# tenpy/tenpy

Hardware: NVIDIA H100
Metric: dmrg_two_site_sweep_wall_clock (lower is better)
Workload: dtype f64

## Files before the change

tenpy_b200/csrc/common.cuh:

```cuda
#pragma once
#include <cuda_runtime.h>
#include <stdint.h>
#include <stdio.h>
#include <atomic>
#include <string>

#include "../../include/b200npc.h"

namespace b200 {

extern thread_local std::string g_last_error;
int set_error(int code, const char *fmt, ...);

#define B200_CUDA_CHECK(expr)                                                                        \
    do {                                                                                             \
        cudaError_t _e = (expr);                                                                     \
        if (_e != cudaSuccess)                                                                       \
            return b200::set_error(B200_ERR_CUDA, "%s failed at %s:%d: %s", #expr, __FILE__, __LINE__, \
                                   cudaGetErrorString(_e));                                          \
    } while (0)

#define B200_CHECK_LAUNCH()                                                                          \
    do {                                                                                             \
        b200::g_kernel_launches.fetch_add(1, std::memory_order_relaxed);                             \
        cudaError_t _e = cudaGetLastError();                                                         \
        if (_e != cudaSuccess)                                                                       \
            return b200::set_error(B200_ERR_CUDA, "kernel launch failed at %s:%d: %s", __FILE__,       \
                                   __LINE__, cudaGetErrorString(_e));                                \
    } while (0)

int sm_count();
extern std::atomic<long long> g_kernel_launches;

#ifndef B200_DMMA_K4
#define B200_DMMA_K4 0
#endif

__device__ __forceinline__ void dmma_m8n8k4(double &c0, double &c1, double a, double b) {
    asm volatile("mma.sync.aligned.m8n8k4.row.col.f64.f64.f64.f64 {%0,%1}, {%2}, {%3}, {%0,%1};\n"
                 : "+d"(c0), "+d"(c1)
                 : "d"(a), "d"(b));
}

__device__ __forceinline__ void dmma_16x8x8_k4(double (&c)[4], const double (&a)[4], const double (&b)[2]) {
    dmma_m8n8k4(c[0], c[1], a[0], b[0]);
    dmma_m8n8k4(c[0], c[1], a[2], b[1]);
    dmma_m8n8k4(c[2], c[3], a[1], b[0]);
    dmma_m8n8k4(c[2], c[3], a[3], b[1]);
}

__device__ __forceinline__ void dmma_16x8x8_k8(double (&c)[4], const double (&a)[4], const double (&b)[2]) {
    asm volatile(
        "mma.sync.aligned.m16n8k8.row.col.f64.f64.f64.f64 {%0,%1,%2,%3}, {%4,%5,%6,%7}, {%8,%9}, "
        "{%0,%1,%2,%3};\n"
        : "+d"(c[0]), "+d"(c[1]), "+d"(c[2]), "+d"(c[3])
        : "d"(a[0]), "d"(a[1]), "d"(a[2]), "d"(a[3]), "d"(b[0]), "d"(b[1]));
}

__device__ __forceinline__ void dmma_16x8x8(double (&c)[4], const double (&a)[4], const double (&b)[2]) {
#if B200_DMMA_K4
    dmma_16x8x8_k4(c, a, b);
#else
    dmma_16x8x8_k8(c, a, b);
#endif
}

__device__ __forceinline__ uint32_t smem_u32(const void *p) {
    return static_cast<uint32_t>(__cvta_generic_to_shared(p));
}
__device__ __forceinline__ void cp_async16(void *smem_dst, const void *gsrc, int src_bytes) {
    asm volatile("cp.async.cg.shared.global [%0], [%1], 16, %2;\n" ::"r"(smem_u32(smem_dst)), "l"(gsrc),
                 "r"(src_bytes));
}
__device__ __forceinline__ void cp_async8(void *smem_dst, const void *gsrc, int src_bytes) {
    asm volatile("cp.async.ca.shared.global [%0], [%1], 8, %2;\n" ::"r"(smem_u32(smem_dst)), "l"(gsrc),
                 "r"(src_bytes));
}
__device__ __forceinline__ void cp_async_commit() { asm volatile("cp.async.commit_group;\n" ::); }
template <int N>
__device__ __forceinline__ void cp_async_wait() {
    asm volatile("cp.async.wait_group %0;\n" ::"n"(N));
}

__device__ __forceinline__ double warp_sum(double v) {
#pragma unroll
    for (int o = 16; o > 0; o >>= 1) v += __shfl_xor_sync(0xffffffffu, v, o);
    return v;
}
__device__ __forceinline__ double warp_max(double v) {
#pragma unroll
    for (int o = 16; o > 0; o >>= 1) v = fmax(v, __shfl_xor_sync(0xffffffffu, v, o));
    return v;
}
__device__ __forceinline__ double block_sum(double v, double *red) {
    v = warp_sum(v);
    int lane = threadIdx.x & 31, w = threadIdx.x >> 5;
    if (lane == 0) red[w] = v;
    __syncthreads();
    int nw = (blockDim.x + 31) >> 5;
    double r = 0.0;
    if (w == 0) {
        r = (lane < nw) ? red[lane] : 0.0;
        r = warp_sum(r);
    }
    __syncthreads();
    return r;
}

}
```

tenpy_b200/csrc/gemm.cu:

```cuda
#include <algorithm>
#include <cstdarg>
#include <cstring>
#include <numeric>
#include <vector>

#include "common.cuh"

namespace b200 {

thread_local std::string g_last_error;
std::atomic<long long> g_kernel_launches{0};

int set_error(int code, const char *fmt, ...) {
    char buf[1024];
    va_list ap;
    va_start(ap, fmt);
    vsnprintf(buf, sizeof(buf), fmt, ap);
    va_end(ap);
    g_last_error = buf;
    return code;
}

int sm_count() {
    static int cached = -1;
    if (cached < 0) {
        int dev = 0, n = 0;
        if (cudaGetDevice(&dev) == cudaSuccess &&
            cudaDeviceGetAttribute(&n, cudaDevAttrMultiProcessorCount, dev) == cudaSuccess)
            cached = n;
        else
            return 132;
    }
    return cached;
}

struct GemmTask {
    int64_t c_off;
    int32_t m, n;
    int32_t pair_begin, pair_end;
};
struct GemmPair {
    int64_t a_off, b_off;
    int32_t k, pad;
};
struct GemmTile {
    int32_t task, tm, tn, pad;
};

constexpr int GEMM_BK = 16;
constexpr int GEMM_STAGES = 3;

template <int BM, int BN>
constexpr int gemm_smem_bytes() {
    return GEMM_STAGES * (BM * (GEMM_BK + 4) + GEMM_BK * (BN + 4)) * (int)sizeof(double);
}

template <int BM, int BN, int WARPS_M, int WARPS_N, bool VEC>
__global__ void __launch_bounds__(WARPS_M *WARPS_N * 32)
    grouped_gemm_kernel(const double *__restrict__ A, const double *__restrict__ B, double *__restrict__ C,
                        const GemmTile *__restrict__ tiles, const GemmTask *__restrict__ tasks,
                        const GemmPair *__restrict__ pairs) {
    constexpr int BK = GEMM_BK, STAGES = GEMM_STAGES;
    constexpr int NTHR = WARPS_M * WARPS_N * 32;
    constexpr int WM = BM / WARPS_M, WN = BN / WARPS_N;
    constexpr int MT = WM / 16, NTL = WN / 8;
    constexpr int LDA_S = BK + 4, LDB_S = BN + 4;
    static_assert(WM % 16 == 0 && WN % 8 == 0, "warp tile");

    extern __shared__ __align__(16) double smem[];
    double *As = smem;
    double *Bs = smem + STAGES * BM * LDA_S;

    const GemmTile tile = tiles[blockIdx.x];
    const GemmTask task = tasks[tile.task];
    const int m = task.m, n = task.n;
    const int row0 = tile.tm * BM, col0 = tile.tn * BN;
    const int tid = threadIdx.x, lane = tid & 31, warp = tid >> 5;
    const int warp_m = warp / WARPS_N, warp_n = warp % WARPS_N;
    const int g = lane >> 2, t = lane & 3;

    int total = 0;
    for (int p = task.pair_begin; p < task.pair_end; ++p) total += (pairs[p].k + BK - 1) / BK;

    int pp = task.pair_begin, pk = 0;
    GemmPair cur = (pp < task.pair_end) ? pairs[pp] : GemmPair{0, 0, 0, 0};

    auto load_stage = [&](int stage) {
        const int k = cur.k;
        const int kbase = pk * BK;
// ... 46 lines not shown
            ++pp;
            if (pp < task.pair_end) cur = pairs[pp];
        }
    };

    double acc[MT][NTL][4];
#pragma unroll
    for (int i = 0; i < MT; ++i)
#pragma unroll
        for (int j = 0; j < NTL; ++j)
#pragma unroll
            for (int e = 0; e < 4; ++e) acc[i][j][e] = 0.0;

    int loaded = 0;
#pragma unroll
    for (int s = 0; s < STAGES - 1; ++s) {
        if (loaded < total) {
            load_stage(s);
            ++loaded;
        }
        cp_async_commit();
    }

    for (int it = 0; it < total; ++it) {
        cp_async_wait<STAGES - 2>();
        __syncthreads();
        if (loaded < total) {
            load_stage((it + STAGES - 1) % STAGES);
            ++loaded;
        }
        cp_async_commit();

        const double *as = As + (it % STAGES) * BM * LDA_S + (warp_m * WM) * LDA_S;
        const double *bs = Bs + (it % STAGES) * BK * LDB_S + warp_n * WN;
#pragma unroll
        for (int kk = 0; kk < BK; kk += 8) {
            double af[MT][4], bf[NTL][2];
#pragma unroll
            for (int i = 0; i < MT; ++i) {
                const double *ap = as + (i * 16 + g) * LDA_S + kk + t;
                af[i][0] = ap[0];
                af[i][1] = ap[8 * LDA_S];
                af[i][2] = ap[4];
                af[i][3] = ap[8 * LDA_S + 4];
            }
#pragma unroll
            for (int j = 0; j < NTL; ++j) {
                const double *bp = bs + (kk + t) * LDB_S + j * 8 + g;
                bf[j][0] = bp[0];
                bf[j][1] = bp[4 * LDB_S];
            }
#pragma unroll
            for (int i = 0; i < MT; ++i)
#pragma unroll
                for (int j = 0; j < NTL; ++j) dmma_16x8x8(acc[i][j], af[i], bf[j]);
        }
    }
    cp_async_wait<0>();

    double *cg = C + task.c_off;
#pragma unroll
    for (int i = 0; i < MT; ++i) {
#pragma unroll
        for (int j = 0; j < NTL; ++j) {
            int r = row0 + warp_m * WM + i * 16 + g;
            int c = col0 + warp_n * WN + j * 8 + 2 * t;
#pragma unroll
            for (int h = 0; h < 2; ++h) {
                int rr = r + 8 * h;
                if (rr < m) {
                    double *dst = cg + (int64_t)rr * n + c;
                    if (VEC) {
                        if (c < n) *reinterpret_cast<double2 *>(dst) = make_double2(acc[i][j][2 * h], acc[i][j][2 * h + 1]);
                    } else {
                        if (c < n) dst[0] = acc[i][j][2 * h];
                        if (c + 1 < n) dst[1] = acc[i][j][2 * h + 1];
                    }
                }
            }
        }
    }
}

constexpr int THIN_MAX = 8;
constexpr int THIN_KSUM = 64;
constexpr int THIN_ROWS = 256;

__global__ void __launch_bounds__(THIN_ROWS)
    thin_n_kernel(const double *__restrict__ A, const double *__restrict__ B, double *__restrict__ C,
                  const GemmTile *__restrict__ tiles, const GemmTask *__restrict__ tasks, const GemmPair *__restrict__ pairs) {
    const GemmTile tile = tiles[blockIdx.x];
    const GemmTask task = tasks[tile.task];
    const int64_t r = (int64_t)tile.tm * THIN_ROWS + threadIdx.x;
    if (r >= task.m) return;
    const int n = task.n;
    double acc[THIN_MAX];
#pragma unroll
    for (int j = 0; j < THIN_MAX; ++j) acc[j] = 0.0;
    for (int p = task.pair_begin; p < task.pair_end; ++p) {
        const GemmPair pr = pairs[p];
        const double *a = A + pr.a_off + r * pr.k;
        const double *b = B + pr.b_off;
        for (int kk = 0; kk < pr.k; ++kk) {
            const double av = a[kk];
#pragma unroll
            for (int j = 0; j < THIN_MAX; ++j)
                if (j < n) acc[j] = fma(av, __ldg(b + (int64_t)kk * n + j), acc[j]);
        }
    }
    double *c = C + task.c_off + r * n;
#pragma unroll
    for (int j = 0; j < THIN_MAX; ++j)
        if (j < n) c[j] = acc[j];
}

__global__ void __launch_bounds__(THIN_ROWS)
    thin_m_kernel(const double *__restrict__ A, const double *__restrict__ B, double *__restrict__ C,
                  const GemmTile *__restrict__ tiles, const GemmTask *__restrict__ tasks, const GemmPair *__restrict__ pairs) {
    const GemmTile tile = tiles[blockIdx.x];
    const GemmTask task = tasks[tile.task];
    const int64_t col = (int64_t)tile.tn * THIN_ROWS + threadIdx.x;
    if (col >= task.n) return;
    const int m = task.m, n = task.n;
    double acc[THIN_MAX];
#pragma unroll
    for (int i = 0; i < THIN_MAX; ++i) acc[i] = 0.0;
    for (int p = task.pair_begin; p < task.pair_end; ++p) {
        const GemmPair pr = pairs[p];
        const double *a = A + pr.a_off;
        const double *b = B + pr.b_off + col;
        for (int kk = 0; kk < pr.k; ++kk) {
            const double bv = b[(int64_t)kk * n];
#pragma unroll
            for (int i = 0; i < THIN_MAX; ++i)
                if (i < m) acc[i] = fma(__ldg(a + (int64_t)i * pr.k + kk), bv, acc[i]);
        }
    }
    double *c = C + task.c_off + col;
#pragma unroll
    for (int i = 0; i < THIN_MAX; ++i)
        if (i < m) c[(int64_t)i * n] = acc[i];
}

struct TileSet {
    std::vector<GemmTile> tiles[5];
};

static inline int64_t cdiv(int64_t a, int64_t b) { return (a + b - 1) / b; }

static void build_tiles(const std::vector<GemmTask> &tasks, const std::vector<GemmPair> &pairs, TileSet &ts) {
    struct Key {
        int64_t work;
        GemmTile tile;
    };
    std::vector<Key> keyed[5];
    static const int force_cfg = getenv("B200_GEMM_FORCE_CFG") ? atoi(getenv("B200_GEMM_FORCE_CFG")) : -1;
    for (size_t ti = 0; ti < tasks.size(); ++ti) {
        const GemmTask &tk = tasks[ti];
        if (tk.m <= 0 || tk.n <= 0) continue;
        int64_t ksum = 0;
        for (int p = tk.pair_begin; p < tk.pair_end; ++p) ksum += pairs[p].k;
        int64_t area128 = cdiv(tk.m, 128) * cdiv(tk.n, 128) * 128 * 128;
        int64_t area64 = cdiv(tk.m, 64) * cdiv(tk.n, 64) * 64 * 64;
        int64_t area32 = cdiv(tk.m, 32) * cdiv(tk.n, 32) * 32 * 32;
        (void)area128;
        int cfg = 1;
        if (area32 * 10 < area64 * 7) cfg = 2;
        if (force_cfg >= 0) cfg = force_cfg;
        if (force_cfg < 0 && ksum <= THIN_KSUM) {
            if (tk.n <= THIN_MAX && tk.m >= 4 * tk.n) cfg = 3;
            else if (tk.m <= THIN_MAX && tk.n >= 4 * tk.m) cfg = 4;
        }
        if (cfg >= 3) {
            int64_t nt = cdiv(cfg == 3 ? tk.m : tk.n, THIN_ROWS);
            for (int64_t i = 0; i < nt; ++i) {
                Key k;
                k.work = ksum;
                k.tile = cfg == 3 ? GemmTile{(int32_t)ti, (int32_t)i, 0, 0} : GemmTile{(int32_t)ti, 0, (int32_t)i, 0};
                keyed[cfg].push_back(k);
            }
            continue;
        }
        int b = cfg == 0 ? 128 : (cfg == 1 ? 64 : 32);
        for (int tm = 0; tm < cdiv(tk.m, b); ++tm)
            for (int tn = 0; tn < cdiv(tk.n, b); ++tn) {
                Key k;
                k.work = ksum;
                k.tile = GemmTile{(int32_t)ti, tm, tn, 0};
                keyed[cfg].push_back(k);
            }
    }
    for (int c = 0; c < 5; ++c) {
        std::stable_sort(keyed[c].begin(), keyed[c].end(), [](const Key &x, const Key &y) { return x.work > y.work; });
        ts.tiles[c].clear();
        for (auto &k : keyed[c]) ts.tiles[c].push_back(k.tile);
    }
}

struct DeviceGemmDesc {
    GemmTask *tasks = nullptr;
    GemmPair *pairs = nullptr;
    GemmTile *tiles[5] = {nullptr, nullptr, nullptr, nullptr, nullptr};
    int n_tiles[5] = {0, 0, 0, 0, 0};
    bool vec = false;
    int device = -1;
    void release() {
        if (tasks) cudaFree(tasks);
        if (pairs) cudaFree(pairs);
        for (int c = 0; c < 5; ++c) {
            if (tiles[c]) cudaFree(tiles[c]);
            tiles[c] = nullptr;
        }
        tasks = nullptr;
        pairs = nullptr;
    }
};

static int upload_desc(const std::vector<GemmTask> &tasks, const std::vector<GemmPair> &pairs, DeviceGemmDesc &d) {
    TileSet ts;
    build_tiles(tasks, pairs, ts);
    B200_CUDA_CHECK(cudaGetDevice(&d.device));
    if (!tasks.empty()) {
        B200_CUDA_CHECK(cudaMalloc(&d.tasks, tasks.size() * sizeof(GemmTask)));
        B200_CUDA_CHECK(cudaMemcpy(d.tasks, tasks.data(), tasks.size() * sizeof(GemmTask), cudaMemcpyHostToDevice));
    }
    if (!pairs.empty()) {
        B200_CUDA_CHECK(cudaMalloc(&d.pairs, pairs.size() * sizeof(GemmPair)));
        B200_CUDA_CHECK(cudaMemcpy(d.pairs, pairs.data(), pairs.size() * sizeof(GemmPair), cudaMemcpyHostToDevice));
    }
    for (int c = 0; c < 5; ++c) {
        d.n_tiles[c] = (int)ts.tiles[c].size();
        if (d.n_tiles[c]) {
            B200_CUDA_CHECK(cudaMalloc(&d.tiles[c], ts.tiles[c].size() * sizeof(GemmTile)));
            B200_CUDA_CHECK(cudaMemcpy(d.tiles[c], ts.tiles[c].data(), ts.tiles[c].size() * sizeof(GemmTile),
                                       cudaMemcpyHostToDevice));
        }
    }
    bool vec = true;
    for (auto &t : tasks)
        if ((t.n & 1) || (t.c_off & 1)) vec = false;
    for (auto &p : pairs)
        if ((p.k & 1) || (p.a_off & 1) || (p.b_off & 1)) vec = false;
    d.vec = vec;
    return B200_OK;
}

template <int BM, int BN, int WMW, int WNW, bool VEC>
static int launch_cfg(const DeviceGemmDesc &d, int cfg, const double *A, const double *B, double *C, cudaStream_t st) {
    if (d.n_tiles[cfg] == 0) return B200_OK;
    auto kern = grouped_gemm_kernel<BM, BN, WMW, WNW, VEC>;
    constexpr int smem = gemm_smem_bytes<BM, BN>();
    static bool attr_set = false;
    if (!attr_set) {
        B200_CUDA_CHECK(cudaFuncSetAttribute(kern, cudaFuncAttributeMaxDynamicSharedMemorySize, smem));
        attr_set = true;
    }
    kern<<<d.n_tiles[cfg], WMW * WNW * 32, smem, st>>>(A, B, C, d.tiles[cfg], d.tasks, d.pairs);
    B200_CHECK_LAUNCH();
    return B200_OK;
}

static int run_desc(const DeviceGemmDesc &d, const double *A, const double *B, double *C, cudaStream_t st) {
    int rc;
    if (d.n_tiles[3]) {
        thin_n_kernel<<<d.n_tiles[3], THIN_ROWS, 0, st>>>(A, B, C, d.tiles[3], d.tasks, d.pairs);
        B200_CHECK_LAUNCH();
    }
    if (d.n_tiles[4]) {
        thin_m_kernel<<<d.n_tiles[4], THIN_ROWS, 0, st>>>(A, B, C, d.tiles[4], d.tasks, d.pairs);
        B200_CHECK_LAUNCH();
    }
    if (d.vec && (((uintptr_t)A | (uintptr_t)B | (uintptr_t)C) & 15) == 0) {
        if ((rc = launch_cfg<128, 128, 2, 4, true>(d, 0, A, B, C, st))) return rc;
        if ((rc = launch_cfg<64, 64, 2, 2, true>(d, 1, A, B, C, st))) return rc;
        if ((rc = launch_cfg<32, 32, 2, 2, true>(d, 2, A, B, C, st))) return rc;
    } else {
        if ((rc = launch_cfg<128, 128, 2, 4, false>(d, 0, A, B, C, st))) return rc;
        if ((rc = launch_cfg<64, 64, 2, 2, false>(d, 1, A, B, C, st))) return rc;
        if ((rc = launch_cfg<32, 32, 2, 2, false>(d, 2, A, B, C, st))) return rc;
    }
    return B200_OK;
}

}

using namespace b200;

struct b200_tdot_plan {
    int32_t rank_c = 0;
    std::vector<int64_t> c_qdata, c_off, c_rows, c_cols;
    std::vector<GemmTask> tasks;
    std::vector<GemmPair> pairs;
    int64_t c_size = 0;
    double flops = 0.0;
    DeviceGemmDesc dev;
    bool uploaded = false;
};

namespace {
struct LexLess {
    const int64_t *base;
    int64_t stride;
    int32_t col0, w;
    bool operator()(int64_t i, int64_t j) const {
        const int64_t *x = base + i * stride + col0, *y = base + j * stride + col0;
        for (int32_t c = w - 1; c >= 0; --c) {
            if (x[c] != y[c]) return x[c] < y[c];
        }
        return false;
    }
    bool equal(int64_t i, int64_t j) const {
        const int64_t *x = base + i * stride + col0, *y = base + j * stride + col0;
        for (int32_t c = 0; c < w; ++c)
            if (x[c] != y[c]) return false;
        return true;
    }
};

void group_ids(const int64_t *tab, int64_t n, int64_t stride, int32_t col0, int32_t w, std::vector<int64_t> &ids,
               std::vector<int64_t> &rep) {
    ids.assign(n, 0);
    rep.clear();
    if (n == 0) return;
    std::vector<int64_t> order(n);
    std::iota(order.begin(), order.end(), 0);
    LexLess less{tab, stride, col0, w};
    if (w > 0) std::stable_sort(order.begin(), order.end(), less);
    int64_t gid = -1;
    for (int64_t i = 0; i < n; ++i) {
        if (i == 0 || (w > 0 && !less.equal(order[i - 1], order[i]))) {
            ++gid;
            rep.push_back(order[i]);
        }
        ids[order[i]] = gid;
    }
}
}

extern "C" int b200_tdot_plan_create(const int64_t *a_qdata, int64_t n_a, int32_t rank_a, const int64_t *b_qdata,
                                     int64_t n_b, int32_t rank_b, int32_t n_contr, const int64_t *a_rows,
                                     const int64_t *a_cols, const int64_t *a_off, const int64_t *b_rows,
                                     const int64_t *b_cols, const int64_t *b_off, b200_tdot_plan **plan_out) {
    if (!plan_out) return set_error(B200_ERR_ARG, "plan_out is NULL");
    if (n_contr < 0 || n_contr > rank_a || n_contr > rank_b) return set_error(B200_ERR_ARG, "bad n_contr");
    const int32_t keep_a = rank_a - n_contr, keep_b = rank_b - n_contr;
    auto *plan = new b200_tdot_plan();
    plan->rank_c = keep_a + keep_b;

    std::vector<int64_t> row_id, row_rep, col_id, col_rep;
    group_ids(a_qdata, n_a, rank_a, 0, keep_a, row_id, row_rep);
    group_ids(b_qdata, n_b, rank_b, n_contr, keep_b, col_id, col_rep);

    std::vector<int64_t> contr(((size_t)n_a + n_b) * (n_contr > 0 ? n_contr : 1));
    for (int64_t i = 0; i < n_a; ++i)
        for (int32_t c = 0; c < n_contr; ++c) contr[i * n_contr + c] = a_qdata[i * rank_a + keep_a + c];
    for (int64_t j = 0; j < n_b; ++j)
        for (int32_t c = 0; c < n_contr; ++c) contr[(n_a + j) * n_contr + c] = b_qdata[j * rank_b + c];
    std::vector<int64_t> kid, krep;
    group_ids(contr.data(), n_a + n_b, n_contr > 0 ? n_contr : 1, 0, n_contr, kid, krep);
    const int64_t n_k = (int64_t)krep.size();
// ... 222 lines not shown
```

tenpy_b200/csrc/ozaki.cu:

```cuda
#include <algorithm>
#include <cstdlib>
#include <vector>

#include "common.cuh"
#include "tc05.cuh"

namespace b200 {

namespace {

constexpr int OZ_MAX_SLICES = 10;
constexpr int OZ_TILE = 128;
constexpr int OZ_CHUNK_BYTES = 16 * OZ_TILE;
constexpr int OZ_SMEM_BUDGET = 224 * 1024;

__host__ __device__ inline int64_t oz_row_tiles(int64_t rows) { return (rows + OZ_TILE - 1) / OZ_TILE; }
__host__ __device__ inline int64_t oz_k_chunks(int64_t k) { return (k + 63) / 64 * 4; }

struct SplitLayout {
    int64_t rt, kc, digits_bytes, scale_off, max_off, total;
};
__host__ inline SplitLayout split_layout(int64_t rows, int64_t k, int slices) {
    SplitLayout L;
    L.rt = oz_row_tiles(rows);
// ... 289 lines not shown
            p.dbg[1] = t_wait;
        }
        return;
    }
    if (warp < 4) return;

    const int cw = (warp >> 2) - 1;
    const int wl = warp & 3;
    uint32_t acc[4][32];
    uint32_t it = 0;
    bool ok = true;
    long long t_full = 0, t_epi = 0, t0 = clock64();
    for (int tile = blockIdx.x; tile < ntiles && ok; tile += gridDim.x) {
        const int mt = tile % mt_count, nt = tile / mt_count;
        for (int g = npass - 1; g >= 0 && ok; --g) {
            const int d_hi = s - 1 - 4 * (npass - 1 - g), d_lo = max(0, d_hi - 3);
            for (int ks = 0; ks < ksteps; ++ks, ++it) {
                const int slot = it % nst;
                const long long tw = clock64();
                ok = mbar_wait(&full_bar[slot], (it / nst) & 1, p.abort_flag);
                t_full += clock64() - tw;
                if (!ok) break;
                const uint32_t sa = smem_addr(oz_smem + (size_t)slot * stage_bytes) + (uint32_t)cw * 64u * 16u;
                const uint32_t sb = smem_addr(oz_smem + (size_t)slot * stage_bytes + (size_t)s * a_bytes);
                wgmma_fence();
                for (int kk = 0; kk < cps / 2; ++kk) {
#pragma unroll
                    for (int j = 0; j < 4; ++j) {
                        const int d = d_lo + j;
                        if (d > d_hi) break;
                        for (int t = 0; t <= d; ++t) {
                            const uint64_t ad = smem_desc(sa + (uint32_t)t * a_bytes + (uint32_t)kk * 2u * OZ_CHUNK_BYTES,
                                                          OZ_CHUNK_BYTES, 128);
                            const uint64_t bd = smem_desc(sb + (uint32_t)(d - t) * b_bytes + (uint32_t)kk * OZ_CHUNK_BYTES,
                                                          OZ_CHUNK_BYTES / 2, 128);
                            wgmma_s8_m64n64k32(acc[j], ad, bd, (ks | kk | t) ? 1u : 0u);
                        }
                    }
                }
                wgmma_commit();
                wgmma_wait_all();
                mbar_arrive(&empty_bar[slot]);
            }
            if (!ok) break;
            const long long te = clock64();
            const int npd = d_hi - d_lo + 1;
            const double wpass = __longlong_as_double((long long)(1023 - 12 - 7 * d_lo) << 52);
            const bool add = (g != npass - 1) || p.accumulate;
            const int row0 = mt * OZ_TILE + cw * 64 + wl * 16 + (lane >> 2);
            const double sa_r[2] = {p.sA[row0], p.sA[row0 + 8]};
#pragma unroll
            for (int j = 0; j < 8; ++j) {
#pragma unroll
                for (int e = 0; e < 2; ++e) {
                    const int col = nt * OZ_TN + 8 * j + 2 * (lane & 3) + e;
                    if (col >= p.N) continue;
                    const double wsb = wpass * p.sB[col];
#pragma unroll
                    for (int hr = 0; hr < 2; ++hr) {
                        const int row = row0 + 8 * hr;
                        if (row >= p.M) continue;
                        const int i = 4 * j + 2 * hr + e;
                        double h = 0.0;
#pragma unroll
                        for (int q = 3; q >= 0; --q)
                            if (q < npd) h = (q == npd - 1) ? oz_i2d(acc[q][i]) : fma(h, 0.0078125, oz_i2d(acc[q][i]));
                        h *= sa_r[hr];
                        double *cp = p.C + (int64_t)row * p.ldc + col;
                        *cp = add ? fma(h, wsb, *cp) : h * wsb;
                    }
                }
            }
            t_epi += clock64() - te;
        }
    }
    if (p.dbg && blockIdx.x == 0 && threadIdx.x == 128) {
        p.dbg[2] = clock64() - t0;
        p.dbg[3] = t_full;
        p.dbg[4] = t_epi;
    }
}

const bool g_split_fused = getenv("B200_OZ_SPLIT2") == nullptr;
int *g_abort_flag = nullptr;
int g_abort_dev = -1;

int ensure_abort_flag() {
    int dev = 0;
    B200_CUDA_CHECK(cudaGetDevice(&dev));
    if (g_abort_flag == nullptr || dev != g_abort_dev) {
        B200_CUDA_CHECK(cudaMalloc(&g_abort_flag, sizeof(int)));
        B200_CUDA_CHECK(cudaMemset(g_abort_flag, 0, sizeof(int)));
        g_abort_dev = dev;
    }
    return B200_OK;
}

}

}

using namespace b200;

extern "C" int64_t b200_ozaki_split_worksize(int64_t rows, int64_t k, int32_t slices) {
    if (rows <= 0 || k <= 0 || slices < 1 || slices > OZ_MAX_SLICES) return 0;
    return split_layout(rows, k, slices).total;
}

extern "C" int b200_ozaki_split_f64(int64_t rows, int64_t k, const double *X, int64_t ld_row, int64_t ld_k,
                                    int32_t slices, void *out_dev, int64_t out_bytes, b200_stream_t stream) {
    if (rows <= 0 || k <= 0) return set_error(B200_ERR_ARG, "ozaki_split: empty operand");
    if (slices < 1 || slices > OZ_MAX_SLICES) return set_error(B200_ERR_ARG, "ozaki_split: slices must be 1..%d", OZ_MAX_SLICES);
    if (ld_row != 1 && ld_k != 1) return set_error(B200_ERR_ARG, "ozaki_split: one of ld_row, ld_k must be 1");
    SplitLayout L = split_layout(rows, k, slices);
    if (out_bytes < L.total) return set_error(B200_ERR_ARG, "ozaki_split: output buffer too small (%lld < %lld)",
                                              (long long)out_bytes, (long long)L.total);
    if (L.kc > 65535) return set_error(B200_ERR_ARG, "ozaki_split: k too large");
    cudaStream_t st = (cudaStream_t)stream;
    uint8_t *base = static_cast<uint8_t *>(out_dev);
    double *scale = reinterpret_cast<double *>(base + L.scale_off);
    unsigned long long *maxbits = reinterpret_cast<unsigned long long *>(base + L.max_off);
    if (slices <= OZ_FUSED_MAX_SLICES && g_split_fused) {
        const unsigned nblk = (unsigned)(L.rt * OZ_TILE / OZF_ROWS);
        if (ld_k == 1)
            oz_split_fused_kernel<true><<<nblk, OZF_THREADS, 0, st>>>(X, rows, k, ld_row, slices, L.rt, L.kc, scale, base);
        else
            oz_split_fused_kernel<false><<<nblk, OZF_THREADS, 0, st>>>(X, rows, k, ld_k, slices, L.rt, L.kc, scale, base);
        B200_CHECK_LAUNCH();
        return B200_OK;
    }
    if (ld_k == 1) {
        int rows_per_block = 8;
        oz_rowmax_kcontig_kernel<<<(unsigned)((rows + rows_per_block - 1) / rows_per_block), 32 * rows_per_block, 0, st>>>(
            X, rows, k, ld_row, maxbits);
        B200_CHECK_LAUNCH();
    } else {
        B200_CUDA_CHECK(cudaMemsetAsync(maxbits, 0, (size_t)L.rt * OZ_TILE * 8, st));
        int64_t ksplit = std::max<int64_t>(1, std::min<int64_t>((k + 255) / 256, 64));
        int64_t k_per_block = (k + ksplit - 1) / ksplit;
        dim3 grid((unsigned)((rows + 31) / 32), (unsigned)ksplit);
        oz_rowmax_rcontig_kernel<<<grid, 256, 0, st>>>(X, rows, k, ld_k, k_per_block, maxbits);
        B200_CHECK_LAUNCH();
    }
    dim3 grid((unsigned)((L.rt * OZ_TILE + 127) / 128), (unsigned)L.kc);
    oz_split_kernel<<<grid, 128, 0, st>>>(X, rows, k, ld_row, ld_k, slices, L.rt, L.kc, maxbits, scale, base);
    B200_CHECK_LAUNCH();
    return B200_OK;
}

extern "C" int b200_ozaki_mm_f64(int64_t m, int64_t n, int64_t k, int32_t slices, const void *a_split,
                                 const void *b_split, double *C, int64_t ldc, int32_t accumulate,
                                 b200_stream_t stream) {
    if (m <= 0 || n <= 0 || k <= 0) return set_error(B200_ERR_ARG, "ozaki_mm: empty product");
    if (slices < 1 || slices > OZ_MAX_SLICES) return set_error(B200_ERR_ARG, "ozaki_mm: slices must be 1..%d", OZ_MAX_SLICES);
    if ((double)oz_k_chunks(k) * 16.0 * 4096.0 * slices >= 2147483648.0)
        return set_error(B200_ERR_ARG, "ozaki_mm: k = %lld too large for exact int32 accumulation with %d slices",
                         (long long)k, slices);
    int rc = ensure_abort_flag();
    if (rc) return rc;
    SplitLayout La = split_layout(m, k, slices), Lb = split_layout(n, k, slices);
    OzGemmArgs p;
    p.As = static_cast<const uint8_t *>(a_split);
    p.Bs = static_cast<const uint8_t *>(b_split);
    p.sA = reinterpret_cast<const double *>(p.As + La.scale_off);
    p.sB = reinterpret_cast<const double *>(p.Bs + Lb.scale_off);
    p.C = C;
    p.ldc = ldc;
    p.M = (int32_t)m;
    p.N = (int32_t)n;
    p.kc = (int32_t)La.kc;
    p.rta = (int32_t)La.rt;
    p.rtb = (int32_t)Lb.rt;
    p.slices = slices;
    p.accumulate = accumulate ? 1 : 0;
    p.abort_flag = g_abort_flag;
    p.dbg = nullptr;
    static const bool debug = getenv("B200_OZ_DEBUG") != nullptr;
    long long *dbg_dev = nullptr;
    if (debug) {
        B200_CUDA_CHECK(cudaMalloc(&dbg_dev, 8 * sizeof(long long)));
        B200_CUDA_CHECK(cudaMemset(dbg_dev, 0, 8 * sizeof(long long)));
        p.dbg = dbg_dev;
    }
    static const int force_cps = getenv("B200_OZ_CPS") ? atoi(getenv("B200_OZ_CPS")) : 0;
    p.cps = force_cps == 2 ? 2 : 4;
    int64_t stage = 3LL * slices * p.cps * (OZ_CHUNK_BYTES / 2);
    if (OZ_SMEM_BUDGET / stage < 2) {
        p.cps = 2;
        stage = 3LL * slices * p.cps * (OZ_CHUNK_BYTES / 2);
    }
    p.nstages = (int32_t)std::min<int64_t>(OZ_MAX_STAGES, OZ_SMEM_BUDGET / stage);
    if (p.nstages < 1) return set_error(B200_ERR_ARG, "ozaki_mm: too many slices for shared memory");
    size_t smem = (size_t)p.nstages * stage;
    static bool attr_set = false;
    if (!attr_set) {
        B200_CUDA_CHECK(cudaFuncSetAttribute(oz_gemm_kernel, cudaFuncAttributeMaxDynamicSharedMemorySize, OZ_SMEM_BUDGET));
        attr_set = true;
    }
    int64_t ntiles = oz_row_tiles(m) * ((n + OZ_TN - 1) / OZ_TN);
    int grid = (int)std::min<int64_t>(ntiles, sm_count());
    oz_gemm_kernel<<<grid, OZ_THREADS, smem, (cudaStream_t)stream>>>(p);
    B200_CHECK_LAUNCH();
    if (debug) {
        long long h[8];
        B200_CUDA_CHECK(cudaMemcpy(h, dbg_dev, sizeof(h), cudaMemcpyDeviceToHost));
        cudaFree(dbg_dev);
        fprintf(stderr, "[oz_gemm m=%lld n=%lld k=%lld s=%d cps=%d stages=%d] CTA0 cycles: producer total %lld wait_empty %lld | "
                "consumer total %lld wait_full %lld epilogue %lld\n",
                (long long)m, (long long)n, (long long)k, slices, p.cps, p.nstages, h[0], h[1], h[2], h[3], h[4]);
    }
    return B200_OK;
}

extern "C" int b200_ozaki_check_abort(void) {
    if (!g_abort_flag) return B200_OK;
    int flag = 0;
    B200_CUDA_CHECK(cudaMemcpy(&flag, g_abort_flag, sizeof(int), cudaMemcpyDeviceToHost));
    if (flag) {
        cudaMemset(g_abort_flag, 0, sizeof(int));
        return set_error(B200_ERR_CUDA, "ozaki kernel: a pipeline wait timed out (watchdog)");
    }
    return B200_OK;
}

extern "C" int64_t b200_ozaki_gemm_worksize(int64_t m, int64_t n, int64_t k, int32_t slices) {
    return b200_ozaki_split_worksize(m, k, slices) + 256 + b200_ozaki_split_worksize(n, k, slices);
}

extern "C" int b200_ozaki_gemm_f64(int64_t m, int64_t n, int64_t k, const double *A, int64_t lda, const double *B,
                                   int64_t ldb, double *C, int64_t ldc, int32_t slices, int32_t accumulate,
                                   void *work_dev, int64_t work_bytes, b200_stream_t stream) {
    int64_t wa = b200_ozaki_split_worksize(m, k, slices), wb = b200_ozaki_split_worksize(n, k, slices);
    if (wa == 0 || wb == 0) return set_error(B200_ERR_ARG, "ozaki_gemm: bad shape or slice count");
    int64_t off_b = (wa + 255) / 256 * 256;
    if (work_bytes < off_b + wb) return set_error(B200_ERR_ARG, "ozaki_gemm: workspace too small");
    uint8_t *w = static_cast<uint8_t *>(work_dev);
    int rc = b200_ozaki_split_f64(m, k, A, lda, 1, slices, w, wa, stream);
    if (rc) return rc;
    rc = b200_ozaki_split_f64(n, k, B, 1, ldb, slices, w + off_b, wb, stream);
    if (rc) return rc;
    return b200_ozaki_mm_f64(m, n, k, slices, w, w + off_b, C, ldc, accumulate, stream);
}
```

tenpy_b200/csrc/tc05.cuh:

```cuda
#pragma once
#include <cuda_runtime.h>
#include <stdint.h>

namespace b200 {
namespace sm90 {

__device__ __forceinline__ uint32_t smem_addr(const void *p) {
    return static_cast<uint32_t>(__cvta_generic_to_shared(p));
}

__device__ __forceinline__ void mbar_init(uint64_t *bar, uint32_t count) {
    asm volatile("mbarrier.init.shared::cta.b64 [%0], %1;\n" ::"r"(smem_addr(bar)), "r"(count) : "memory");
}
__device__ __forceinline__ void mbar_fence_init() {
    asm volatile("fence.mbarrier_init.release.cluster;\n" ::: "memory");
}
__device__ __forceinline__ void mbar_expect_tx(uint64_t *bar, uint32_t bytes) {
    asm volatile("mbarrier.arrive.expect_tx.shared::cta.b64 _, [%0], %1;\n" ::"r"(smem_addr(bar)), "r"(bytes)
                 : "memory");
}
__device__ __forceinline__ void mbar_arrive(uint64_t *bar) {
    asm volatile("mbarrier.arrive.shared::cta.b64 _, [%0];\n" ::"r"(smem_addr(bar)) : "memory");
}
__device__ __forceinline__ bool mbar_try_wait(uint64_t *bar, uint32_t parity) {
    uint32_t ok;
    asm volatile(
        "{\n\t.reg .pred p;\n\t"
        "mbarrier.try_wait.parity.shared::cta.b64 p, [%1], %2;\n\t"
        "selp.u32 %0, 1, 0, p;\n\t}\n"
        : "=r"(ok)
        : "r"(smem_addr(bar)), "r"(parity)
        : "memory");
    return ok != 0;
}
__device__ __forceinline__ bool mbar_wait(uint64_t *bar, uint32_t parity, volatile int *abort_flag,
                                          uint32_t limit = 1u << 26) {
    for (uint32_t it = 0; it < limit; ++it) {
        if (mbar_try_wait(bar, parity)) return true;
        if ((it & 1023u) == 1023u && *abort_flag) return false;
    }
    *abort_flag = 1;
    return false;
}

__device__ __forceinline__ void bulk_g2s(void *smem_dst, const void *gsrc, uint32_t bytes, uint64_t *bar) {
    asm volatile(
        "cp.async.bulk.shared::cluster.global.mbarrier::complete_tx::bytes [%0], [%1], %2, [%3];\n" ::"r"(
            smem_addr(smem_dst)),
        "l"(gsrc), "r"(bytes), "r"(smem_addr(bar))
        : "memory");
}

__device__ __forceinline__ uint64_t smem_desc(uint32_t saddr, uint32_t lbo_bytes, uint32_t sbo_bytes) {
    uint64_t d = 0;
    d |= (uint64_t)((saddr >> 4) & 0x3FFF);
    d |= (uint64_t)((lbo_bytes >> 4) & 0x3FFF) << 16;
    d |= (uint64_t)((sbo_bytes >> 4) & 0x3FFF) << 32;
    return d;
}

__device__ __forceinline__ void wgmma_fence() { asm volatile("wgmma.fence.sync.aligned;\n" ::: "memory"); }
__device__ __forceinline__ void wgmma_commit() { asm volatile("wgmma.commit_group.sync.aligned;\n" ::: "memory"); }
__device__ __forceinline__ void wgmma_wait_all() { asm volatile("wgmma.wait_group.sync.aligned 0;\n" ::: "memory"); }

__device__ __forceinline__ void wgmma_s8_m64n64k32(uint32_t (&d)[32], uint64_t a_desc, uint64_t b_desc,
                                                   uint32_t accumulate) {
    asm volatile(
        "{\n\t.reg .pred p;\n\t"
        "setp.ne.b32 p, %34, 0;\n\t"
        "wgmma.mma_async.sync.aligned.m64n64k32.s32.s8.s8 "
        "{%0,%1,%2,%3,%4,%5,%6,%7,%8,%9,%10,%11,%12,%13,%14,%15,"
        "%16,%17,%18,%19,%20,%21,%22,%23,%24,%25,%26,%27,%28,%29,%30,%31}, %32, %33, p;\n\t}\n"
        : "+r"(d[0]), "+r"(d[1]), "+r"(d[2]), "+r"(d[3]), "+r"(d[4]), "+r"(d[5]), "+r"(d[6]), "+r"(d[7]), "+r"(d[8]),
          "+r"(d[9]), "+r"(d[10]), "+r"(d[11]), "+r"(d[12]), "+r"(d[13]), "+r"(d[14]), "+r"(d[15]), "+r"(d[16]),
          "+r"(d[17]), "+r"(d[18]), "+r"(d[19]), "+r"(d[20]), "+r"(d[21]), "+r"(d[22]), "+r"(d[23]), "+r"(d[24]),
          "+r"(d[25]), "+r"(d[26]), "+r"(d[27]), "+r"(d[28]), "+r"(d[29]), "+r"(d[30]), "+r"(d[31])
        : "l"(a_desc), "l"(b_desc), "r"(accumulate)
        : "memory");
}

}
}
```

Before: 3.809.

## Add warp-specialized persistent 128x128 FP64 GEMM with mbarrier pipeline

```diff
diff --git a/profiles/gemm_h100.py b/profiles/gemm_h100.py
--- /dev/null
+++ b/profiles/gemm_h100.py
@@ -0,0 +1,125 @@
+#!/usr/bin/env python
+import argparse
+import json
+import os
+import subprocess
+import sys
+
+import numpy as np
+import torch
+
+ROOT = os.path.dirname(os.path.dirname(os.path.abspath(__file__)))
+sys.path.insert(0, ROOT)
+from tenpy_b200._lib import DeviceLib
+
+SHAPES = {
+    'matvec 1': (2048, 4096, 1024), 'matvec 2': (4096, 1024, 2048),
+    'env LHeff': (6144, 1024, 2048), 'env RHeff': (1024, 3072, 2048),
+    'newton-schulz kf^2 x 2048': (901, 901, 2048), 'newton-schulz kf x 2048 x kf': (901, 2048, 901),
+}
+GROUPED = {
+    '48 x (256, 256, 256)': [(256, 256, 256)] * 48,
+    '48 x (256, 256, 128)': [(256, 256, 128)] * 48,
+    '12 x (512, 512, 512)': [(512, 512, 512)] * 12,
+    '(1536, 1536, 256)': [(1536, 1536, 256)],
+    '(1024, 1024, 1024)': [(1024, 1024, 1024)],
+}
+
+
+def card():
+    q = 'name,power.limit,power.max_limit,clocks.sm,clocks.max.sm,temperature.gpu'
+    try:
+        out = subprocess.run(['nvidia-smi', '--query-gpu=' + q, '--format=csv,noheader'], capture_output=True, text=True,
+                             timeout=60).stdout.strip().splitlines()[0]
+        return dict(zip(q.split(','), [s.strip() for s in out.split(',')]))
+    except Exception as e:
+        return {'error': repr(e)}
+
+
+def timed(fn, reps, warmup):
+    for _ in range(warmup):
+        fn()
+    torch.cuda.synchronize()
+    ev = [(torch.cuda.Event(enable_timing=True), torch.cuda.Event(enable_timing=True)) for _ in range(reps)]
+    for e0, e1 in ev:
+        e0.record()
+        fn()
+        e1.record()
+    torch.cuda.synchronize()
+    ms = np.array([e0.elapsed_time(e1) for e0, e1 in ev])
+    return {'median_ms': float(np.median(ms)), 'min_ms': float(ms.min()), 'max_ms': float(ms.max()), 'reps': reps}
+
+
+def grouped_args(blocks):
+    m = [b[0] for b in blocks]
+    n = [b[1] for b in blocks]
+    k = [b[2] for b in blocks]
+    a_off = np.concatenate(([0], np.cumsum([(x * y + 15) // 16 * 16 for x, y in zip(m, k)])))
+    b_off = np.concatenate(([0], np.cumsum([(x * y + 15) // 16 * 16 for x, y in zip(k, n)])))
+    c_off = np.concatenate(([0], np.cumsum([(x * y + 15) // 16 * 16 for x, y in zip(m, n)])))
+    return (m, n, c_off[:-1], np.arange(len(blocks) + 1), k, a_off[:-1], b_off[:-1]), a_off[-1], b_off[-1], c_off[-1]
+
+
+def main():
+    ap = argparse.ArgumentParser()
+    ap.add_argument('--other-lib', default=None, help='a second build of libb200npc.so to time next to this tree\'s')
+    ap.add_argument('--reps', type=int, default=25)
+    ap.add_argument('--warmup', type=int, default=5)
+    ap.add_argument('--out', default=None, help='also write the JSON document to this file')
+    args = ap.parse_args()
+    assert torch.cuda.is_available(), 'needs a CUDA device'
+    libs = {'this': DeviceLib()}
+    if args.other_lib:
+        libs['other'] = DeviceLib(args.other_lib)
+    dev = libs['this'].device
+    res = {'card_before': card(), 'torch': torch.__version__, 'shapes': {}, 'grouped': {}}
+    g = torch.Generator(device=dev).manual_seed(0)
+    for name, (m, n, k) in SHAPES.items():
+        A = torch.randn(m, k, dtype=torch.float64, device=dev, generator=g)
+        B = torch.randn(k, n, dtype=torch.float64, device=dev, generator=g)
+        flop = 2. * m * n * k
+        row = {'m': m, 'n': n, 'k': k}
+        Cref = A @ B
+        for tag, lib in libs.items():
+            gg, _, _, csz = grouped_args([(m, n, k)])
+            C = torch.empty(int(csz), dtype=torch.float64, device=dev)
+            Af, Bf = A.reshape(-1), B.reshape(-1)
+            row[tag] = timed(lambda: lib.grouped_gemm(*gg, Af, Bf, C), args.reps, args.warmup)
+            row[tag]['tflops'] = flop / row[tag]['median_ms'] / 1e9
+            row[tag]['max_rel_diff_vs_cublas'] = float((C[:m * n].reshape(m, n) - Cref).abs().max() / Cref.abs().max())
+        Ct = torch.empty(m, n, dtype=torch.float64, device=dev)
+        row['cublas'] = timed(lambda: torch.matmul(A, B, out=Ct), args.reps, args.warmup)
+        row['cublas']['tflops'] = flop / row['cublas']['median_ms'] / 1e9
+        row['this_frac_of_cublas'] = row['cublas']['median_ms'] / row['this']['median_ms']
+        if 'other' in row:
+            row['speedup_vs_other'] = row['other']['median_ms'] / row['this']['median_ms']
+        res['shapes'][name] = row
+        print(json.dumps({name: row}), flush=True)
+    for name, blocks in GROUPED.items():
+        gg, asz, bsz, csz = grouped_args(blocks)
+        A = torch.randn(int(asz), dtype=torch.float64, device=dev, generator=g)
+        B = torch.randn(int(bsz), dtype=torch.float64, device=dev, generator=g)
+        flop = sum(2. * m * n * k for m, n, k in blocks)
+        row = {}
+        outs = {}
+        for tag, lib in libs.items():
+            C = torch.zeros(int(csz), dtype=torch.float64, device=dev)
+            row[tag] = timed(lambda: lib.grouped_gemm(*gg, A, B, C), args.reps, args.warmup)
+            row[tag]['tflops'] = flop / row[tag]['median_ms'] / 1e9
+            outs[tag] = C
+        if 'other' in row:
+            row['speedup_vs_other'] = row['other']['median_ms'] / row['this']['median_ms']
+            row['max_abs_diff_vs_other'] = float((outs['this'] - outs['other']).abs().max())
+        res['grouped'][name] = row
+        print(json.dumps({name: row}), flush=True)
+    libs['this'].ozaki_check_abort()
+    res['card_after'] = card()
+    if args.out:
+        os.makedirs(os.path.dirname(os.path.abspath(args.out)), exist_ok=True)
+        with open(args.out, 'w') as f:
+            json.dump(res, f, indent=1)
+    print(json.dumps(res))
+
+
+if __name__ == '__main__':
+    main()
diff --git a/tenpy_b200/csrc/common.cuh b/tenpy_b200/csrc/common.cuh
--- a/tenpy_b200/csrc/common.cuh
+++ b/tenpy_b200/csrc/common.cuh
@@ -30,6 +30,8 @@
     } while (0)
 
 int sm_count();
+extern int *g_abort_flag;
+int ensure_abort_flag();
 extern std::atomic<long long> g_kernel_launches;
 
 #ifndef B200_DMMA_K4
@@ -63,6 +65,15 @@
 #else
     dmma_16x8x8_k8(c, a, b);
 #endif
+}
+
+__device__ __forceinline__ void dmma_16x8x16(double (&c)[4], const double (&a)[8], const double (&b)[4]) {
+    asm volatile(
+        "mma.sync.aligned.m16n8k16.row.col.f64.f64.f64.f64 {%0,%1,%2,%3}, {%4,%5,%6,%7,%8,%9,%10,%11}, "
+        "{%12,%13,%14,%15}, {%0,%1,%2,%3};\n"
+        : "+d"(c[0]), "+d"(c[1]), "+d"(c[2]), "+d"(c[3])
+        : "d"(a[0]), "d"(a[1]), "d"(a[2]), "d"(a[3]), "d"(a[4]), "d"(a[5]), "d"(a[6]), "d"(a[7]), "d"(b[0]), "d"(b[1]),
+          "d"(b[2]), "d"(b[3]));
 }
 
 __device__ __forceinline__ uint32_t smem_u32(const void *p) {
diff --git a/tenpy_b200/csrc/gemm.cu b/tenpy_b200/csrc/gemm.cu
--- a/tenpy_b200/csrc/gemm.cu
+++ b/tenpy_b200/csrc/gemm.cu
@@ -5,6 +5,7 @@
 #include <vector>
 
 #include "common.cuh"
+#include "tc05.cuh"
 
 namespace b200 {
 
@@ -217,6 +218,147 @@
     }
 }
 
+constexpr int G0_BM = 128, G0_BN = 128, G0_BK = 16, G0_STAGES = 6;
+constexpr int G0_LDA = G0_BK + 4, G0_LDB = G0_BN + 4;
+constexpr int G0_CONSUMER_WARPS = 8;
+constexpr int G0_PRODUCER_THREADS = 128;
+constexpr int G0_THREADS = G0_CONSUMER_WARPS * 32 + G0_PRODUCER_THREADS;
+constexpr int G0_STAGE = G0_BM * G0_LDA + G0_BK * G0_LDB;
+constexpr int G0_SMEM = G0_STAGES * G0_STAGE * (int)sizeof(double);
+constexpr int G0_MIN_KSUM = 256;
+constexpr int G0_BAND = 8;
+
+template <bool VEC>
+__global__ void __launch_bounds__(G0_THREADS, 1)
+    gemm128_kernel(const double *__restrict__ A, const double *__restrict__ B, double *__restrict__ C,
+                   const GemmTile *__restrict__ tiles, int n_tiles, const GemmTask *__restrict__ tasks,
+                   const GemmPair *__restrict__ pairs, int *abort_flag) {
+    using namespace sm90;
+    extern __shared__ __align__(16) double smem[];
+    __shared__ uint64_t full_bar[G0_STAGES], empty_bar[G0_STAGES];
+    const int warp = threadIdx.x >> 5, lane = threadIdx.x & 31;
+    if (threadIdx.x == 0) {
+        for (int s = 0; s < G0_STAGES; ++s) {
+            mbar_init(&full_bar[s], G0_PRODUCER_THREADS);
+            mbar_init(&empty_bar[s], G0_CONSUMER_WARPS);
+        }
+        mbar_fence_init();
+    }
+    __syncthreads();
+
+    if (warp >= G0_CONSUMER_WARPS) {
+        asm volatile("setmaxnreg.dec.sync.aligned.u32 56;\n" ::: "memory");
+        const int pt = threadIdx.x - G0_CONSUMER_WARPS * 32;
+        constexpr int W = VEC ? 2 : 1;
+        constexpr int A_RSTEP = G0_PRODUCER_THREADS / (G0_BK / W);
+        constexpr int B_RSTEP = G0_PRODUCER_THREADS / (G0_BN / W);
+        const int a_r = pt / (G0_BK / W), a_c = pt % (G0_BK / W) * W;
+        const int b_r = pt / (G0_BN / W), b_c = pt % (G0_BN / W) * W;
+        auto copy = [](double *dst, const double *src, bool ok) {
+            if (VEC) cp_async16(dst, src, ok ? 16 : 0);
+            else cp_async8(dst, src, ok ? 8 : 0);
+        };
+        uint32_t it = 0;
+        for (int ti = blockIdx.x; ti < n_tiles; ti += gridDim.x) {
+            const GemmTile tile = tiles[ti];
+            const GemmTask task = tasks[tile.task];
+            const int m = task.m, n = task.n;
+            const int row0 = tile.tm * G0_BM, col0 = tile.tn * G0_BN;
+            for (int p = task.pair_begin; p < task.pair_end; ++p) {
+                const GemmPair pr = pairs[p];
+                const int k = pr.k;
+                const double *ag = A + pr.a_off;
+                const double *bg = B + pr.b_off;
+                for (int kb = 0; kb < k; kb += G0_BK, ++it) {
+                    const int slot = it % G0_STAGES;
+                    if (!mbar_wait(&empty_bar[slot], ((it / G0_STAGES) & 1) ^ 1, abort_flag)) return;
+                    double *as = smem + slot * G0_STAGE;
+                    double *bs = as + G0_BM * G0_LDA;
+                    const int ac = kb + a_c, bc = col0 + b_c;
+                    const double *asrc = ag + (int64_t)(row0 + a_r) * k + ac;
+                    const double *bsrc = bg + (int64_t)(kb + b_r) * n + bc;
+#pragma unroll 4
+                    for (int r = 0; r < G0_BM; r += A_RSTEP) {
+                        const bool ok = (ac < k) && (row0 + a_r + r < m);
+                        copy(as + (a_r + r) * G0_LDA + a_c, ok ? asrc + (int64_t)r * k : ag, ok);
+                    }
+#pragma unroll 4
+                    for (int r = 0; r < G0_BK; r += B_RSTEP) {
+                        const bool ok = (bc < n) && (kb + b_r + r < k);
+                        copy(bs + (b_r + r) * G0_LDB + b_c, ok ? bsrc + (int64_t)r * n : bg, ok);
+                    }
+                    mbar_cp_async_arrive(&full_bar[slot]);
+                }
+            }
+        }
+        return;
+    }
+
+    asm volatile("setmaxnreg.inc.sync.aligned.u32 224;\n" ::: "memory");
+    const int wm = warp >> 2, wn = warp & 3;
+    const int g = lane >> 2, t = lane & 3;
+    uint32_t it = 0;
+    for (int ti = blockIdx.x; ti < n_tiles; ti += gridDim.x) {
+        const GemmTile tile = tiles[ti];
+        const GemmTask task = tasks[tile.task];
+        const int m = task.m, n = task.n;
+        const int row0 = tile.tm * G0_BM, col0 = tile.tn * G0_BN;
+        double acc[4][4][4];
+#pragma unroll
+        for (int i = 0; i < 4; ++i)
+#pragma unroll
+            for (int j = 0; j < 4; ++j)
+#pragma unroll
+                for (int e = 0; e < 4; ++e) acc[i][j][e] = 0.0;
+        for (int p = task.pair_begin; p < task.pair_end; ++p) {
+            const int k = pairs[p].k;
+            for (int kb = 0; kb < k; kb += G0_BK, ++it) {
+                const int slot = it % G0_STAGES;
+                if (!mbar_wait(&full_bar[slot], (it / G0_STAGES) & 1, abort_flag)) return;
+                const double *as = smem + slot * G0_STAGE + (wm * 64 + g) * G0_LDA + t;
+                const double *bs = smem + slot * G0_STAGE + G0_BM * G0_LDA + t * G0_LDB + wn * 32 + g;
+                double bf[4][4];
+#pragma unroll
+                for (int j = 0; j < 4; ++j)
+#pragma unroll
+                    for (int q = 0; q < 4; ++q) bf[j][q] = bs[4 * q * G0_LDB + 8 * j];
+#pragma unroll
+                for (int i = 0; i < 4; ++i) {
+                    double af[8];
+#pragma unroll
+                    for (int q = 0; q < 8; ++q) af[q] = as[(16 * i + 8 * (q & 1)) * G0_LDA + 4 * (q >> 1)];
+#pragma unroll
+                    for (int j = 0; j < 4; ++j) dmma_16x8x16(acc[i][j], af, bf[j]);
+                }
+                __syncwarp();
+                if (lane == 0) mbar_arrive(&empty_bar[slot]);
+            }
+        }
+        double *cg = C + task.c_off;
+#pragma unroll
+        for (int i = 0; i < 4; ++i) {
+#pragma unroll
+            for (int j = 0; j < 4; ++j) {
+                const int r = row0 + wm * 64 + i * 16 + g;
+                const int c = col0 + wn * 32 + j * 8 + 2 * t;
+#pragma unroll
+                for (int h = 0; h < 2; ++h) {
+                    const int rr = r + 8 * h;
+                    if (rr < m) {
+                        double *dst = cg + (int64_t)rr * n + c;
+                        if (VEC) {
+                            if (c < n) *reinterpret_cast<double2 *>(dst) = make_double2(acc[i][j][2 * h], acc[i][j][2 * h + 1]);
+                        } else {
+                            if (c < n) dst[0] = acc[i][j][2 * h];
+                            if (c + 1 < n) dst[1] = acc[i][j][2 * h + 1];
+                        }
+                    }
+                }
+            }
+        }
+    }
+}
+
 constexpr int THIN_MAX = 8;
 constexpr int THIN_KSUM = 64;
 constexpr int THIN_ROWS = 256;
@@ -290,17 +432,24 @@
     };
     std::vector<Key> keyed[5];
     static const int force_cfg = getenv("B200_GEMM_FORCE_CFG") ? atoi(getenv("B200_GEMM_FORCE_CFG")) : -1;
+    std::vector<int64_t> ksums(tasks.size(), 0);
+    auto large = [&](const GemmTask &tk, int64_t ksum) { return tk.m >= G0_BM && tk.n >= G0_BN && ksum >= G0_MIN_KSUM; };
+    int64_t tiles128 = 0;
+    for (size_t ti = 0; ti < tasks.size(); ++ti) {
+        const GemmTask &tk = tasks[ti];
+        for (int p = tk.pair_begin; p < tk.pair_end; ++p) ksums[ti] += pairs[p].k;
+        if (large(tk, ksums[ti])) tiles128 += cdiv(tk.m, G0_BM) * cdiv(tk.n, G0_BN);
+    }
+    const bool use128 = tiles128 >= sm_count();
     for (size_t ti = 0; ti < tasks.size(); ++ti) {
         const GemmTask &tk = tasks[ti];
         if (tk.m <= 0 || tk.n <= 0) continue;
-        int64_t ksum = 0;
-        for (int p = tk.pair_begin; p < tk.pair_end; ++p) ksum += pairs[p].k;
-        int64_t area128 = cdiv(tk.m, 128) * cdiv(tk.n, 128) * 128 * 128;
+        const int64_t ksum = ksums[ti];
         int64_t area64 = cdiv(tk.m, 64) * cdiv(tk.n, 64) * 64 * 64;
         int64_t area32 = cdiv(tk.m, 32) * cdiv(tk.n, 32) * 32 * 32;
-        (void)area128;
         int cfg = 1;
         if (area32 * 10 < area64 * 7) cfg = 2;
+        if (use128 && large(tk, ksum)) cfg = 0;
         if (force_cfg >= 0) cfg = force_cfg;
         if (force_cfg < 0 && ksum <= THIN_KSUM) {
             if (tk.n <= THIN_MAX && tk.m >= 4 * tk.n) cfg = 3;
@@ -316,7 +465,15 @@
             }
             continue;
         }
-        int b = cfg == 0 ? 128 : (cfg == 1 ? 64 : 32);
+        if (cfg == 0) {
+            const int mt = (int)cdiv(tk.m, G0_BM), nt = (int)cdiv(tk.n, G0_BN);
+            for (int band = 0; band < mt; band += G0_BAND)
+                for (int tn = 0; tn < nt; ++tn)
+                    for (int tm = band; tm < std::min(mt, band + G0_BAND); ++tm)
+                        keyed[0].push_back(Key{ksum, GemmTile{(int32_t)ti, tm, tn, 0}});
+            continue;
+        }
+        int b = cfg == 1 ? 64 : 32;
         for (int tm = 0; tm < cdiv(tk.m, b); ++tm)
             for (int tn = 0; tn < cdiv(tk.n, b); ++tn) {
                 Key k;
@@ -395,6 +552,23 @@
     return B200_OK;
 }
 
+template <bool VEC>
+static int launch_128(const DeviceGemmDesc &d, const double *A, const double *B, double *C, cudaStream_t st) {
+    if (d.n_tiles[0] == 0) return B200_OK;
+    int rc = ensure_abort_flag();
+    if (rc) return rc;
+    static bool attr_set = false;
+    if (!attr_set) {
+        B200_CUDA_CHECK(cudaFuncSetAttribute(gemm128_kernel<VEC>, cudaFuncAttributeMaxDynamicSharedMemorySize, G0_SMEM));
+        attr_set = true;
+    }
+    const int grid = std::min(d.n_tiles[0], sm_count());
+    gemm128_kernel<VEC><<<grid, G0_THREADS, G0_SMEM, st>>>(A, B, C, d.tiles[0], d.n_tiles[0], d.tasks, d.pairs,
+                                                           g_abort_flag);
+    B200_CHECK_LAUNCH();
+    return B200_OK;
+}
+
 static int run_desc(const DeviceGemmDesc &d, const double *A, const double *B, double *C, cudaStream_t st) {
     int rc;
     if (d.n_tiles[3]) {
@@ -406,11 +580,11 @@
         B200_CHECK_LAUNCH();
     }
     if (d.vec && (((uintptr_t)A | (uintptr_t)B | (uintptr_t)C) & 15) == 0) {
-        if ((rc = launch_cfg<128, 128, 2, 4, true>(d, 0, A, B, C, st))) return rc;
+        if ((rc = launch_128<true>(d, A, B, C, st))) return rc;
         if ((rc = launch_cfg<64, 64, 2, 2, true>(d, 1, A, B, C, st))) return rc;
         if ((rc = launch_cfg<32, 32, 2, 2, true>(d, 2, A, B, C, st))) return rc;
     } else {
-        if ((rc = launch_cfg<128, 128, 2, 4, false>(d, 0, A, B, C, st))) return rc;
+        if ((rc = launch_128<false>(d, A, B, C, st))) return rc;
         if ((rc = launch_cfg<64, 64, 2, 2, false>(d, 1, A, B, C, st))) return rc;
         if ((rc = launch_cfg<32, 32, 2, 2, false>(d, 2, A, B, C, st))) return rc;
     }
diff --git a/tenpy_b200/csrc/ozaki.cu b/tenpy_b200/csrc/ozaki.cu
--- a/tenpy_b200/csrc/ozaki.cu
+++ b/tenpy_b200/csrc/ozaki.cu
@@ -395,8 +395,11 @@
 }
 
 const bool g_split_fused = getenv("B200_OZ_SPLIT2") == nullptr;
+int g_abort_dev = -1;
+
+}
+
 int *g_abort_flag = nullptr;
-int g_abort_dev = -1;
 
 int ensure_abort_flag() {
     int dev = 0;
@@ -407,8 +410,6 @@
         g_abort_dev = dev;
     }
     return B200_OK;
-}
-
 }
 
 }
@@ -531,7 +532,7 @@
     B200_CUDA_CHECK(cudaMemcpy(&flag, g_abort_flag, sizeof(int), cudaMemcpyDeviceToHost));
     if (flag) {
         cudaMemset(g_abort_flag, 0, sizeof(int));
-        return set_error(B200_ERR_CUDA, "ozaki kernel: a pipeline wait timed out (watchdog)");
+        return set_error(B200_ERR_CUDA, "ozaki or 128 x 128 gemm kernel: a pipeline wait timed out (watchdog)");
     }
     return B200_OK;
 }
diff --git a/tenpy_b200/csrc/tc05.cuh b/tenpy_b200/csrc/tc05.cuh
--- a/tenpy_b200/csrc/tc05.cuh
+++ b/tenpy_b200/csrc/tc05.cuh
@@ -21,6 +21,9 @@
 }
 __device__ __forceinline__ void mbar_arrive(uint64_t *bar) {
     asm volatile("mbarrier.arrive.shared::cta.b64 _, [%0];\n" ::"r"(smem_addr(bar)) : "memory");
+}
+__device__ __forceinline__ void mbar_cp_async_arrive(uint64_t *bar) {
+    asm volatile("cp.async.mbarrier.arrive.noinc.shared::cta.b64 [%0];\n" ::"r"(smem_addr(bar)) : "memory");
 }
 __device__ __forceinline__ bool mbar_try_wait(uint64_t *bar, uint32_t parity) {
     uint32_t ok;
```

Result: faster. 3.411 (median of 6 runs) (-10.4%).
